# cloneofsimo/paint-with-words-sd

Hardware: NVIDIA H100
Metric: unet_steps_per_sec_512sq_cfg (higher is better)
Workload: dtype f16

## Files before the change

paint_with_words_sd_b200/csrc/pww_abi.cu:

```cuda
#include <stdio.h>
#include <string.h>

#include "pww_common.cuh"
#include "xattn_tc.cuh"
#include "xattn_fused2.cuh"
#include "attn_tc.cuh"
#include "unet_ops.cuh"
#include "sampler_step.cuh"
#include "control_inject.cuh"
#include "control_combine.cuh"
#include <stdlib.h>
#include <algorithm>
#include <type_traits>

namespace {

thread_local char g_last_cuda_error[640] = "";

int cuda_fail(cudaError_t e);

bool aligned16(const void* p) { return (reinterpret_cast<uintptr_t>(p) & 15u) == 0; }

bool supported_head_dim(int D) { return D == 40 || D == 64 || D == 80 || D == 160; }

// ... 143 lines not shown
              int64_t q_batch_stride, int64_t q_row_stride, int64_t k_batch_stride, int64_t k_row_stride,
              int64_t o_batch_stride, int64_t o_row_stride, const float* wmap, int64_t wmap_batch_stride,
              const int32_t* wmap_index, const float* stats, const float* g_sigma, int64_t g_stride, float scale,
              void* stream) {
  int rc = check_common(q, k, B, H, N, T, D, q_batch_stride, q_row_stride, k_batch_stride, k_row_stride);
  if (rc) return rc;
  if (!v || !out || !aligned16(v) || !aligned16(out)) return PWW_ERR_BAD_ARG;
  if ((o_batch_stride | o_row_stride) & 7 || o_row_stride < (int64_t)H * D) return PWW_ERR_BAD_ARG;
  if (wmap && (!stats || !g_sigma)) return PWW_ERR_BAD_ARG;
  pww::XattnParams<E> p = xattn_params<E>(q, k, v, out, B, H, N, T, D, q_batch_stride, q_row_stride, k_batch_stride,
                                          k_row_stride, o_batch_stride, o_row_stride);
  p.wmap = wmap; p.wmap_bs = wmap_batch_stride; p.wmap_index = wmap ? wmap_index : nullptr;
  p.stats = stats; p.g_sigma = g_sigma; p.g_stride = g_stride; p.scale = scale;
  for (int b0 = 0; b0 < B; b0 += pww::tc::kMaxBatch) {
    pww::XattnParams<E> c = images(p, b0, std::min(B - b0, pww::tc::kMaxBatch));
    if (wmap && !wmap_index) c.wmap += (int64_t)b0 * wmap_batch_stride;
    const cudaError_t e =
        with_shape(D, T, [&](auto k) { return pww::tc::launch_fwd<k.D, k.KC>(c, (cudaStream_t)stream); });
    if (e != cudaSuccess) return cuda_fail(e);
  }
  return PWW_OK;
}

template <typename E>
int xattn_fused(const void* q, const void* k, const void* v, void* out, int B, int H, int N, int T, int D,
                int64_t q_batch_stride, int64_t q_row_stride, int64_t k_batch_stride, int64_t k_row_stride,
                int64_t o_batch_stride, int64_t o_row_stride, const void* mpack, int64_t mpack_batch_stride, int Bw,
                const int8_t* cidx, const int32_t* wmap_index, int stat, const int32_t* kinds, bool per_image,
                const float* g_sigma, float scale, float* stats, void* workspace, size_t workspace_bytes,
                void* stream) {
  int rc = check_common(q, k, B, H, N, T, D, q_batch_stride, q_row_stride, k_batch_stride, k_row_stride);
  if (rc) return rc;
  if (!v || !out || !aligned16(v) || !aligned16(out)) return PWW_ERR_BAD_ARG;
  if ((o_batch_stride | o_row_stride) & 7 || o_row_stride < (int64_t)H * D || o_batch_stride <= 0) return PWW_ERR_BAD_ARG;
  if (mpack) {
    if (!cidx || !g_sigma || !workspace || Bw <= 0 || !aligned16(mpack)) return PWW_ERR_BAD_ARG;
    if ((mpack_batch_stride & 7) || mpack_batch_stride < (int64_t)N * pww::fx::kMW) return PWW_ERR_BAD_ARG;
    if (per_image ? !kinds : (stat != PWW_STAT_MAX && stat != PWW_STAT_STD)) return PWW_ERR_BAD_ARG;
    if (workspace_bytes < pww_xattn_fused_workspace_bytes()) return PWW_ERR_WORKSPACE;
  }
  pww::XattnParams<E> p = xattn_params<E>(q, k, v, out, B, H, N, T, D, q_batch_stride, q_row_stride, k_batch_stride,
                                          k_row_stride, o_batch_stride, o_row_stride);
  p.g_sigma = g_sigma; p.g_stride = per_image ? 1 : 0; p.scale = scale; p.stat = stat;
  p.stat_kind = per_image ? kinds : nullptr; p.stats_out = stats;
  p.wmap_index = mpack ? wmap_index : nullptr;
  p.counters = (unsigned int*)workspace;
  p.partials = workspace ? (pww::StatPartial*)((char*)workspace + 512) : nullptr;
  int chunk = pww::fx::kMaxBatch;
  const int tiles = pww::ceil_div(N, pww::core::kBM);
  const int hg = pww::ceil_div(H, D == 40 ? pww::fx::Cfg2<40>::G : (D == 64 ? pww::fx::Cfg2<64>::G : 1));
  while (chunk > 1) {
    const int cb = B < chunk ? B : chunk;
    if (pww::fx::fused2_fits(cb, hg, tiles, pww::fx::fused_grid(cb * hg * tiles))) break;
    chunk >>= 1;
  }
  for (int b0 = 0; b0 < B; b0 += chunk) {
    pww::XattnParams<E> c = images(p, b0, std::min(B - b0, chunk));
    const void* mp = mpack;
    const int8_t* ci = cidx;
    if (mpack && !wmap_index) {
      mp = (const __half*)mpack + (int64_t)b0 * mpack_batch_stride;
      ci = cidx + (int64_t)b0 * pww::core::kTP * pww::core::chunks_of(T);
    }
    c.wmap = (const float*)mp;
    const cudaError_t e = with_shape(D, T, [&](auto k) {
      return pww::fx::launch_fused2<k.D, k.KC>(c, mp, mpack_batch_stride, ci, (cudaStream_t)stream);
    });
    if (e == cudaErrorInvalidConfiguration) return PWW_ERR_UNSUPPORTED;
    if (e != cudaSuccess) return cuda_fail(e);
  }
  return PWW_OK;
}

template <typename E>
int groupnorm_nhwc(const void* x, const void* add, int64_t add_batch_stride, const void* gamma, const void* beta, void* y,
                   int B, int HW, int C, int G, float eps, int silu, void* workspace, size_t workspace_bytes,
                   void* stream) {
  if (!x || !gamma || !beta || !y || !workspace || B <= 0 || HW <= 0 || C <= 0 || G <= 0) return PWW_ERR_BAD_ARG;
  if (!aligned16(x) || !aligned16(y) || !aligned16(gamma) || !aligned16(beta) || (add && !aligned16(add)))
    return PWW_ERR_BAD_ARG;
  if ((C & 7) || (C % G) || G > 64 || (C >> 3) > 1024) return PWW_ERR_UNSUPPORTED;
  if (add && ((add_batch_stride & 7) || add_batch_stride < C)) return PWW_ERR_BAD_ARG;
  if (workspace_bytes < pww_groupnorm_workspace_bytes(B, HW, G)) return PWW_ERR_WORKSPACE;
  pww::uops::GnParams<E> p;
  p.x = (const E*)x; p.add = (const E*)add; p.add_bs = add_batch_stride; p.gamma = (const E*)gamma; p.beta = (const E*)beta;
  p.y = (E*)y;
  char* w = (char*)workspace;
  p.counters = (unsigned int*)w;
  w += align_up((size_t)B * sizeof(unsigned int), 256);
  p.stats = (float*)w;
  w += align_up((size_t)B * G * 2 * sizeof(float), 256);
  p.partial = (float*)w;
  p.B = B; p.HW = HW; p.C = C; p.G = G; p.eps = eps; p.silu = silu;
  p.chunks = pww::uops::gn_chunks(HW);
  p.rows_per_chunk = (HW + p.chunks - 1) / p.chunks;
  cudaStream_t s = (cudaStream_t)stream;
  const int nvec = C >> 3;
  const int rpp = nvec >= 256 ? 1 : 256 / nvec;
  const size_t smem1 = (size_t)rpp * C * 2 * sizeof(float);
  if (smem1 > 48 * 1024) return PWW_ERR_UNSUPPORTED;
  pww::uops::gn_stats_kernel<E><<<dim3(p.chunks, B), nvec * rpp, smem1, s>>>(p);
  int rows_per_block = (int)(((long long)HW * B + 2 * pww::num_sms() - 1) / (2 * pww::num_sms()));
  if (rows_per_block < rpp) rows_per_block = rpp;
  if (rows_per_block > 32) rows_per_block = 32;
  pww::uops::gn_apply_kernel<E><<<dim3((HW + rows_per_block - 1) / rows_per_block, B), nvec * rpp, 0, s>>>(p, rows_per_block);
  cudaError_t e = cudaGetLastError();
  return e == cudaSuccess ? PWW_OK : cuda_fail(e);
}

template <typename E>
int geglu(const void* in, void* out, int64_t M, int I, void* stream) {
  if (!in || !out || M <= 0 || I <= 0 || !aligned16(in) || !aligned16(out)) return PWW_ERR_BAD_ARG;
  if (I & 7) return PWW_ERR_UNSUPPORTED;
  const long long total = (long long)M * (I >> 3);
  long long blocks = (total + 255) / 256;
  const long long cap = (long long)pww::num_sms() * 16;
  if (blocks > cap) blocks = cap;
  pww::uops::geglu_kernel<E><<<(int)blocks, 256, 0, (cudaStream_t)stream>>>((const E*)in, (E*)out, M, I);
  cudaError_t e = cudaGetLastError();
  return e == cudaSuccess ? PWW_OK : cuda_fail(e);
}

template <typename E>
int add_layernorm(const void* x, const void* res, const void* gamma, const void* beta, void* sum_out, void* y, int64_t M,
                  int C, float eps, void* stream) {
  if (!x || !gamma || !beta || !y || M <= 0 || C <= 0) return PWW_ERR_BAD_ARG;
  if (!aligned16(x) || !aligned16(y) || !aligned16(gamma) || !aligned16(beta) || (res && !aligned16(res)) ||
      (sum_out && !aligned16(sum_out)))
    return PWW_ERR_BAD_ARG;
  if ((C & 7) || C > 2048) return PWW_ERR_UNSUPPORTED;
  const int warps = 8;
  const unsigned grid = (unsigned)((M + warps - 1) / warps);
  with_int<1, 8>(((C >> 3) + 31) / 32, [&](auto vpl) {
    pww::uops::add_layernorm_kernel<E, vpl><<<grid, warps * 32, 0, (cudaStream_t)stream>>>(
        (const E*)x, (const E*)res, (const E*)gamma, (const E*)beta, (E*)sum_out, (E*)y, M, C, eps);
  });
  cudaError_t e = cudaGetLastError();
  return e == cudaSuccess ? PWW_OK : cuda_fail(e);
}

template <typename E>
int resnet_residual(const void* a, const void* h, const float* bias, void* out, int64_t rows, int C, void* stream) {
  if (!a || !h || !bias || !out || rows <= 0 || C <= 0 || (C & 7)) return PWW_ERR_BAD_ARG;
  if (!aligned16(a) || !aligned16(h) || !aligned16(bias) || !aligned16(out)) return PWW_ERR_BAD_ARG;
  const long long total = (long long)rows * (C >> 3);
  long long blocks = (total + 255) / 256;
  const long long cap = (long long)pww::num_sms() * 16;
  if (blocks > cap) blocks = cap;
  pww::uops::resnet_residual_kernel<E><<<(int)blocks, 256, 0, (cudaStream_t)stream>>>(
      (const E*)a, (const E*)h, bias, (E*)out, total, C >> 3);
  cudaError_t e = cudaGetLastError();
  return e == cudaSuccess ? PWW_OK : cuda_fail(e);
}

template <typename E>
int attn_fwd(const void* q,const void* k, const void* v, void* out, int B, int H, int N, int D, int64_t qkv_batch_stride,
             int64_t qkv_row_stride, int64_t o_batch_stride, int64_t o_row_stride, float scale, void* stream) {
  if (!q || !k || !v || !out || B <= 0 || H <= 0 || N <= 0 || D <= 0) return PWW_ERR_BAD_ARG;
  if (!aligned16(q) || !aligned16(k) || !aligned16(v) || !aligned16(out)) return PWW_ERR_BAD_ARG;
  if ((qkv_batch_stride | qkv_row_stride | o_batch_stride | o_row_stride) & 7) return PWW_ERR_BAD_ARG;
  if (qkv_row_stride < (int64_t)H * D || o_row_stride < (int64_t)H * D) return PWW_ERR_BAD_ARG;
  if (!supported_head_dim(D)) return PWW_ERR_UNSUPPORTED;
  const cudaError_t e = with_shape(D, 1, [&](auto sh) {
    return pww::fa::launch<sh.D, E>(q, k, v, out, B, H, N, qkv_batch_stride, qkv_row_stride, o_batch_stride,
                                    o_row_stride, scale, (cudaStream_t)stream);
  });
  return e == cudaSuccess ? PWW_OK : cuda_fail(e);
}

template <typename E>
int control_inject(int n, void* const* dst, const void* const* res, const int64_t* elems_per_image, int rows,
                   const float* scales, void* stream) {
  if (n < 1 || n > pww::ctl::kMaxLevels || rows < 1 || !dst || !res || !elems_per_image) return PWW_ERR_BAD_ARG;
  pww::ctl::InjectArgs a;
  a.off[0] = 0;
  for (int k = 0; k < n; ++k) {
    const int64_t e = elems_per_image[k];
    if (e <= 0 || (e % pww::ctl::kVec) != 0) return PWW_ERR_BAD_ARG;
    if (!dst[k] || !res[k] || !aligned16(dst[k]) || !aligned16(res[k])) return PWW_ERR_BAD_ARG;
    a.dst[k] = dst[k];
    a.res[k] = res[k];
    a.vec_per_image[k] = e / pww::ctl::kVec;
    a.off[k + 1] = a.off[k] + (int64_t)rows * a.vec_per_image[k];
  }
  for (int k = n; k < pww::ctl::kMaxLevels; ++k) {
    a.dst[k] = nullptr;
    a.res[k] = nullptr;
    a.vec_per_image[k] = 0;
    a.off[k + 1] = a.off[n];
// ... 76 lines not shown
}
int pww_xattn_fwd_bf16(const void* q, const void* k, const void* v, void* out, int B, int H, int N, int T, int D,
    int64_t q_batch_stride, int64_t q_row_stride, int64_t k_batch_stride, int64_t k_row_stride, int64_t o_batch_stride,
    int64_t o_row_stride, const float* wmap, int64_t wmap_batch_stride, const int32_t* wmap_index, const float* stats,
    const float* g_sigma, float scale, void* stream) {
  return xattn_fwd<__nv_bfloat16>(
      q, k, v, out, B, H, N, T, D, q_batch_stride, q_row_stride, k_batch_stride, k_row_stride,
      o_batch_stride, o_row_stride, wmap, wmap_batch_stride, wmap_index, stats, g_sigma, 0, scale, stream);
}

int pww_xattn_fwd_multi_f16(const void* q, const void* k, const void* v, void* out, int B, int H, int N, int T, int D,
    int64_t q_batch_stride, int64_t q_row_stride, int64_t k_batch_stride, int64_t k_row_stride, int64_t o_batch_stride,
    int64_t o_row_stride, const float* wmap, int64_t wmap_batch_stride, const int32_t* wmap_index, const float* stats,
    const float* g_sigma, float scale, void* stream) {
  return xattn_fwd<__half>(q, k, v, out, B, H, N, T, D, q_batch_stride, q_row_stride, k_batch_stride, k_row_stride,
      o_batch_stride, o_row_stride, wmap, wmap_batch_stride, wmap_index, stats, g_sigma, 1, scale, stream);
}
int pww_xattn_fwd_multi_bf16(const void* q, const void* k, const void* v, void* out, int B, int H, int N, int T, int D,
    int64_t q_batch_stride, int64_t q_row_stride, int64_t k_batch_stride, int64_t k_row_stride, int64_t o_batch_stride,
    int64_t o_row_stride, const float* wmap, int64_t wmap_batch_stride, const int32_t* wmap_index, const float* stats,
    const float* g_sigma, float scale, void* stream) {
  return xattn_fwd<__nv_bfloat16>(
      q, k, v, out, B, H, N, T, D, q_batch_stride, q_row_stride, k_batch_stride, k_row_stride,
      o_batch_stride, o_row_stride, wmap, wmap_batch_stride, wmap_index, stats, g_sigma, 1, scale, stream);
}

size_t pww_xattn_fused_workspace_bytes(void) { return pww::fx::fused_workspace_bytes(); }

int pww_xattn_fused_f16(const void* q, const void* k, const void* v, void* out, int B, int H, int N, int T, int D,
    int64_t q_batch_stride, int64_t q_row_stride, int64_t k_batch_stride, int64_t k_row_stride, int64_t o_batch_stride,
    int64_t o_row_stride, const void* mpack, int64_t mpack_batch_stride, int Bw, const int8_t* cidx,
    const int32_t* wmap_index, int stat, const float* g_sigma, float scale, float* stats, void* workspace,
    size_t workspace_bytes, void* stream) {
  return xattn_fused<__half>(q, k, v, out, B, H, N, T, D, q_batch_stride, q_row_stride, k_batch_stride, k_row_stride,
      o_batch_stride, o_row_stride, mpack, mpack_batch_stride, Bw, cidx, wmap_index, stat, nullptr, false,
      g_sigma, scale, stats, workspace, workspace_bytes, stream);
}
int pww_xattn_fused_bf16(const void* q, const void* k, const void* v, void* out, int B, int H, int N, int T, int D,
    int64_t q_batch_stride, int64_t q_row_stride, int64_t k_batch_stride, int64_t k_row_stride, int64_t o_batch_stride,
    int64_t o_row_stride, const void* mpack, int64_t mpack_batch_stride, int Bw, const int8_t* cidx,
    const int32_t* wmap_index, int stat, const float* g_sigma, float scale, float* stats, void* workspace,
    size_t workspace_bytes, void* stream) {
  return xattn_fused<__nv_bfloat16>(
      q, k, v, out, B, H, N, T, D, q_batch_stride, q_row_stride, k_batch_stride, k_row_stride,
      o_batch_stride, o_row_stride, mpack, mpack_batch_stride, Bw, cidx, wmap_index, stat, nullptr, false,
      g_sigma, scale, stats, workspace, workspace_bytes, stream);
}

int pww_xattn_fused_multi_f16(const void* q, const void* k, const void* v, void* out, int B, int H, int N, int T, int D,
    int64_t q_batch_stride, int64_t q_row_stride, int64_t k_batch_stride, int64_t k_row_stride, int64_t o_batch_stride,
    int64_t o_row_stride, const void* mpack, int64_t mpack_batch_stride, int Bw, const int8_t* cidx,
    const int32_t* wmap_index, const int32_t* stat, const float* g_sigma, float scale, float* stats, void* workspace,
    size_t workspace_bytes, void* stream) {
  return xattn_fused<__half>(q, k, v, out, B, H, N, T, D, q_batch_stride, q_row_stride, k_batch_stride, k_row_stride,
      o_batch_stride, o_row_stride, mpack, mpack_batch_stride, Bw, cidx, wmap_index, PWW_STAT_MAX, stat, true,
      g_sigma, scale, stats, workspace, workspace_bytes, stream);
}
int pww_xattn_fused_multi_bf16(const void* q, const void* k, const void* v, void* out, int B, int H, int N, int T, int D,
    int64_t q_batch_stride, int64_t q_row_stride, int64_t k_batch_stride, int64_t k_row_stride, int64_t o_batch_stride,
    int64_t o_row_stride, const void* mpack, int64_t mpack_batch_stride, int Bw, const int8_t* cidx,
    const int32_t* wmap_index, const int32_t* stat, const float* g_sigma, float scale, float* stats, void* workspace,
    size_t workspace_bytes, void* stream) {
  return xattn_fused<__nv_bfloat16>(
      q, k, v, out, B, H, N, T, D, q_batch_stride, q_row_stride, k_batch_stride, k_row_stride,
      o_batch_stride, o_row_stride, mpack, mpack_batch_stride, Bw, cidx, wmap_index, PWW_STAT_MAX, stat, true,
      g_sigma, scale, stats, workspace, workspace_bytes, stream);
}

int pww_attn_fwd_f16(const void* q, const void* k, const void* v, void* out, int B, int H, int N, int D,
    int64_t qkv_batch_stride, int64_t qkv_row_stride, int64_t o_batch_stride, int64_t o_row_stride, float scale,
    void* stream) {
  return attn_fwd<__half>(
      q, k, v, out, B, H, N, D, qkv_batch_stride, qkv_row_stride, o_batch_stride, o_row_stride, scale, stream);
}
int pww_attn_fwd_bf16(const void* q, const void* k, const void* v, void* out, int B, int H, int N, int D,
    int64_t qkv_batch_stride, int64_t qkv_row_stride, int64_t o_batch_stride, int64_t o_row_stride, float scale,
    void* stream) {
  return attn_fwd<__nv_bfloat16>(
      q, k, v, out, B, H, N, D, qkv_batch_stride, qkv_row_stride, o_batch_stride, o_row_stride, scale, stream);
}

size_t pww_groupnorm_workspace_bytes(int B, int HW, int G) {
  if (B <= 0 || HW <= 0 || G <= 0) return 0;
  return align_up((size_t)B * sizeof(unsigned int), 256) + align_up((size_t)B * G * 2 * sizeof(float), 256) +
         (size_t)B * pww::uops::gn_chunks(HW) * G * 2 * sizeof(float);
}

int pww_groupnorm_nhwc_f16(const void* x, const void* add, int64_t add_batch_stride, const void* gamma,
    const void* beta, void* y, int B, int HW, int C, int G, float eps, int silu, void* workspace, size_t workspace_bytes,
    void* stream) {
  return groupnorm_nhwc<__half>(
      x, add, add_batch_stride, gamma, beta, y, B, HW, C, G, eps, silu, workspace, workspace_bytes,
      stream);
}
int pww_groupnorm_nhwc_bf16(const void* x, const void* add, int64_t add_batch_stride, const void* gamma,
    const void* beta, void* y, int B, int HW, int C, int G, float eps, int silu, void* workspace, size_t workspace_bytes,
    void* stream) {
  return groupnorm_nhwc<__nv_bfloat16>(
      x, add, add_batch_stride, gamma, beta, y, B, HW, C, G, eps, silu, workspace, workspace_bytes,
      stream);
}

int pww_geglu_f16(const void* in, void* out, int64_t M, int I, void* stream) {
  return geglu<__half>(in, out, M, I, stream);
}
int pww_geglu_bf16(const void* in, void* out, int64_t M, int I, void* stream) {
  return geglu<__nv_bfloat16>(in, out, M, I, stream);
}

int pww_add_layernorm_f16(const void* x, const void* res, const void* gamma, const void* beta, void* sum_out, void* y,
    int64_t M, int C, float eps, void* stream) {
  return add_layernorm<__half>(x, res, gamma, beta, sum_out, y, M, C, eps, stream);
}
int pww_add_layernorm_bf16(const void* x, const void* res, const void* gamma, const void* beta, void* sum_out, void* y,
    int64_t M, int C, float eps, void* stream) {
  return add_layernorm<__nv_bfloat16>(x, res, gamma, beta, sum_out, y, M, C, eps, stream);
}

int pww_resnet_residual_f16(const void* a, const void* h, const float* bias, void* out, int64_t rows, int C,
                            void* stream) {
  return resnet_residual<__half>(a, h, bias, out, rows, C, stream);
}
int pww_resnet_residual_bf16(const void* a, const void* h, const float* bias, void* out, int64_t rows, int C,
                             void* stream) {
  return resnet_residual<__nv_bfloat16>(a, h, bias, out, rows, C, stream);
}

int pww_sampler_input(const float* latents, const float* scale, const float* extra, void* out, int out_dtype, int m,
                      int channels, int height, int width, void* stream) {
  if (!latents || !scale || !out || m <= 0 || height <= 0 || width <= 0) return PWW_ERR_BAD_ARG;
  if (channels != 4 && channels != 9) return PWW_ERR_BAD_ARG;
  if ((channels == 9) != (extra != nullptr)) return PWW_ERR_BAD_ARG;
  if (out_dtype != PWW_DTYPE_F32 && out_dtype != PWW_DTYPE_F16 && out_dtype != PWW_DTYPE_BF16) return PWW_ERR_UNSUPPORTED;
  pww::smp::InputArgs a;
  a.lat = latents; a.scale = scale; a.extra = extra; a.out = out; a.m = m; a.C = channels; a.hw = height * width;
  const bool px4 = (a.hw % 4) == 0 && aligned16(latents) && (!extra || aligned16(extra)) && aligned16(out);
  cudaStream_t s = (cudaStream_t)stream;
  const cudaError_t e = out_dtype == PWW_DTYPE_F16    ? pww::smp::launch_input<__half>(a, px4, s)
                        : out_dtype == PWW_DTYPE_BF16 ? pww::smp::launch_input<__nv_bfloat16>(a, px4, s)
                                                      : pww::smp::launch_input<float>(a, px4, s);
  return e == cudaSuccess ? PWW_OK : cuda_fail(e);
}

int pww_sampler_update(const void* eps, int eps_dtype, int64_t eps_batch_stride, int64_t eps_channel_stride,
                       int64_t eps_row_stride, int64_t eps_col_stride, float* latents, float* history, int history_len,
                       const float* noise, const float* guidance, const float* beta, const float* form, int m,
                       int height, int width, void* stream) {
  if (!eps || !latents || !history || !guidance || !beta || !form) return PWW_ERR_BAD_ARG;
  if (m <= 0 || height <= 0 || width <= 0 || history_len < 1 || history_len > 4) return PWW_ERR_BAD_ARG;
  if (eps_dtype != PWW_DTYPE_F32 && eps_dtype != PWW_DTYPE_F16 && eps_dtype != PWW_DTYPE_BF16) return PWW_ERR_UNSUPPORTED;
  pww::smp::UpdateArgs a;
  a.eps = eps; a.e_sn = eps_batch_stride; a.e_sc = eps_channel_stride; a.e_sh = eps_row_stride; a.e_sw = eps_col_stride;
  a.lat = latents; a.hist = history; a.noise = noise; a.gscale = guidance; a.beta = beta; a.form = form;
  a.m = m; a.h = height; a.w = width; a.nh = history_len;
  const int64_t hw = (int64_t)height * width;
  const size_t es = eps_dtype == PWW_DTYPE_F32 ? 4 : 2;
  const bool px4 = (hw % 4) == 0 && aligned16(latents) && aligned16(history) && (!noise || aligned16(noise));
  const size_t need = px4 ? 16 : 4 * es;
  const bool cl = eps_channel_stride == 1 && eps_col_stride == 4 && eps_row_stride == 4 * (int64_t)width &&
                  (reinterpret_cast<uintptr_t>(eps) % need) == 0 && ((size_t)eps_batch_stride * es) % need == 0;
  cudaStream_t s = (cudaStream_t)stream;
  const cudaError_t e = eps_dtype == PWW_DTYPE_F16    ? pww::smp::launch_update<__half>(a, px4, cl, s)
                        : eps_dtype == PWW_DTYPE_BF16 ? pww::smp::launch_update<__nv_bfloat16>(a, px4, cl, s)
                                                      : pww::smp::launch_update<float>(a, px4, cl, s);
  return e == cudaSuccess ? PWW_OK : cuda_fail(e);
}

int pww_control_inject_f16(int n, void* const* dst, const void* const* res, const int64_t* elems_per_image, int rows,
// ... 42 lines not shown
```

paint_with_words_sd_b200/csrc/unet_ops.cuh:

```cuda
#pragma once
#include "pww_common.cuh"

namespace pww {
namespace uops {

template <typename E>
struct GnParams {
  const E* x;
  const E* add;
  long long add_bs;
  const E* gamma;
  const E* beta;
  E* y;
  float* partial;
  float* stats;
  unsigned int* counters;
  int B, HW, C, G, chunks, rows_per_chunk, silu;
  float eps;
};

template <typename E>
__global__ void gn_stats_kernel(GnParams<E> p) {
  using X = Elem<E>;
  using E2 = typename X::E2;
  extern __shared__ float sm[];
  const int nvec = p.C >> 3;
  const int rpp = blockDim.x / nvec;
  const int v = threadIdx.x % nvec, rl = threadIdx.x / nvec;
  const int b = blockIdx.y, chunk = blockIdx.x;
  const int r0 = chunk * p.rows_per_chunk, r1 = min(p.HW, r0 + p.rows_per_chunk);
  float s[8], q[8], a[8];
#pragma unroll
  for (int i = 0; i < 8; ++i) { s[i] = 0.f; q[i] = 0.f; a[i] = 0.f; }
  if (p.add) {
    const uint4 av = *reinterpret_cast<const uint4*>(p.add + (size_t)b * p.add_bs + v * 8);
    const E2* ah = reinterpret_cast<const E2*>(&av);
#pragma unroll
    for (int i = 0; i < 4; ++i) { float2 f = X::to_float2(ah[i]); a[2 * i] = f.x; a[2 * i + 1] = f.y; }
  }
  const E* xb = p.x + (size_t)b * p.HW * p.C;
  for (int r = r0 + rl; r < r1; r += 4 * rpp) {
    uint4 xv[4];
#pragma unroll
    for (int u = 0; u < 4; ++u) {
      const int rr = r + u * rpp;
      xv[u] = rr < r1 ? __ldg(reinterpret_cast<const uint4*>(xb + (size_t)rr * p.C) + v) : make_uint4(0, 0, 0, 0);
    }
#pragma unroll
    for (int u = 0; u < 4; ++u) {
      if (r + u * rpp < r1) {
        const E2* xh = reinterpret_cast<const E2*>(&xv[u]);
#pragma unroll
        for (int i = 0; i < 4; ++i) {
          float2 f = X::to_float2(xh[i]);
          const float x0 = f.x + a[2 * i], x1 = f.y + a[2 * i + 1];
          s[2 * i] += x0; q[2 * i] = fmaf(x0, x0, q[2 * i]);
          s[2 * i + 1] += x1; q[2 * i + 1] = fmaf(x1, x1, q[2 * i + 1]);
        }
      }
    }
  }
  float* ss = sm;
  float* sq = sm + rpp * p.C;
#pragma unroll
  for (int i = 0; i < 8; ++i) { ss[rl * p.C + v * 8 + i] = s[i]; sq[rl * p.C + v * 8 + i] = q[i]; }
  __syncthreads();
  const int cg = p.C / p.G;
  for (int g = threadIdx.x; g < p.G; g += blockDim.x) {
    float ts = 0.f, tq = 0.f;
    for (int r = 0; r < rpp; ++r)
      for (int c = g * cg; c < (g + 1) * cg; ++c) { ts += ss[r * p.C + c]; tq += sq[r * p.C + c]; }
    float* out = p.partial + (((size_t)b * p.chunks + chunk) * p.G + g) * 2;
    out[0] = ts; out[1] = tq;
  }
  __shared__ int is_last;
  __threadfence();
  __syncthreads();
  if (threadIdx.x == 0) is_last = (atomicAdd(&p.counters[b], 1u) == (unsigned)p.chunks - 1u) ? 1 : 0;
  __syncthreads();
  if (!is_last) return;
  __threadfence();
  const int warp = threadIdx.x >> 5, lane = threadIdx.x & 31, nwarps = blockDim.x >> 5;
  for (int g = warp; warp < nwarps && g < p.G; g += nwarps) {
    const float* pp = p.partial + ((size_t)b * p.chunks * p.G + g) * 2;
    float ts = 0.f, tq = 0.f;
    for (int c = lane; c < p.chunks; c += 32) { ts += __ldcg(pp + (size_t)c * p.G * 2); tq += __ldcg(pp + (size_t)c * p.G * 2 + 1); }
#pragma unroll
    for (int o = 16; o > 0; o >>= 1) {
      ts += __shfl_xor_sync(0xffffffffu, ts, o);
      tq += __shfl_xor_sync(0xffffffffu, tq, o);
    }
    if (lane == 0) {
      const float n = (float)p.HW * (float)cg;
      const float mean = ts / n;
      float var = tq / n - mean * mean;
      var = var < 0.f ? 0.f : var;
      p.stats[((size_t)b * p.G + g) * 2] = mean;
      p.stats[((size_t)b * p.G + g) * 2 + 1] = rsqrtf(var + p.eps);
    }
  }
  if (threadIdx.x == 0) p.counters[b] = 0u;
}

template <typename E>
__global__ void gn_apply_kernel(GnParams<E> p, int rows_per_block) {
  using X = Elem<E>;
  using E2 = typename X::E2;
  const int nvec = p.C >> 3;
  const int rpp = blockDim.x / nvec;
  const int v = threadIdx.x % nvec, rl = threadIdx.x / nvec;
  const int b = blockIdx.y;
  const int cg = p.C / p.G;
  float sc[8], sh[8];
  {
    const uint4 gv = __ldg(reinterpret_cast<const uint4*>(p.gamma) + v);
    const uint4 bv = __ldg(reinterpret_cast<const uint4*>(p.beta) + v);
    uint4 av = make_uint4(0, 0, 0, 0);
    if (p.add) av = __ldg(reinterpret_cast<const uint4*>(p.add + (size_t)b * p.add_bs) + v);
    const E* gh = reinterpret_cast<const E*>(&gv);
    const E* bh = reinterpret_cast<const E*>(&bv);
    const E* ah = reinterpret_cast<const E*>(&av);
#pragma unroll
    for (int i = 0; i < 8; ++i) {
      const int g = (v * 8 + i) / cg;
      const float mean = __ldg(p.stats + ((size_t)b * p.G + g) * 2), rstd = __ldg(p.stats + ((size_t)b * p.G + g) * 2 + 1);
      sc[i] = rstd * X::to_float(gh[i]);
      sh[i] = X::to_float(bh[i]) + (X::to_float(ah[i]) - mean) * sc[i];
    }
  }
  const int r0 = blockIdx.x * rows_per_block, r1 = min(p.HW, r0 + rows_per_block);
  const E* xb = p.x + (size_t)b * p.HW * p.C;
  E* yb = p.y + (size_t)b * p.HW * p.C;
  for (int r = r0 + rl; r < r1; r += rpp) {
    const uint4 xv = __ldg(reinterpret_cast<const uint4*>(xb + (size_t)r * p.C) + v);
    const E2* xh = reinterpret_cast<const E2*>(&xv);
    __align__(16) E2 o[4];
#pragma unroll
    for (int k = 0; k < 4; ++k) {
      const float2 f = X::to_float2(xh[k]);
      float y0 = fmaf(f.x, sc[2 * k], sh[2 * k]);
      float y1 = fmaf(f.y, sc[2 * k + 1], sh[2 * k + 1]);
      if (p.silu) {
        y0 = __fdividef(y0, 1.f + __expf(-y0));
        y1 = __fdividef(y1, 1.f + __expf(-y1));
      }
      o[k] = X::from_float2(y0, y1);
    }
    reinterpret_cast<uint4*>(yb + (size_t)r * p.C)[v] = *reinterpret_cast<const uint4*>(o);
  }
}

template <typename E>
__global__ void geglu_kernel(const E* __restrict__ in, E* __restrict__ out, long long M, int I) {
  using X = Elem<E>;
  using E2 = typename X::E2;
  const int nvec = I >> 3;
  const long long total = M * nvec;
  for (long long i = (long long)blockIdx.x * blockDim.x + threadIdx.x; i < total; i += (long long)gridDim.x * blockDim.x) {
    const long long m = i / nvec;
    const int v = (int)(i % nvec);
    const uint4 av = __ldg(reinterpret_cast<const uint4*>(in + m * 2 * I) + v);
    const uint4 gv = __ldg(reinterpret_cast<const uint4*>(in + m * 2 * I + I) + v);
    const E2* ah = reinterpret_cast<const E2*>(&av);
    const E2* gh = reinterpret_cast<const E2*>(&gv);
    __align__(16) E2 o[4];
#pragma unroll
    for (int k = 0; k < 4; ++k) {
      const float2 a = X::to_float2(ah[k]), g = X::to_float2(gh[k]);
      const float g0 = 0.5f * g.x * (1.f + erff(g.x * 0.70710678118654752f));
      const float g1 = 0.5f * g.y * (1.f + erff(g.y * 0.70710678118654752f));
      o[k] = X::from_float2(a.x * g0, a.y * g1);
    }
    reinterpret_cast<uint4*>(out + m * I)[v] = *reinterpret_cast<const uint4*>(o);
  }
}

template <typename E, int VPL>
__global__ void add_layernorm_kernel(const E* __restrict__ x, const E* __restrict__ res,
                                     const E* __restrict__ gamma, const E* __restrict__ beta,
                                     E* __restrict__ sum_out, E* __restrict__ y, long long M, int C, float eps) {
  using X = Elem<E>;
  using E2 = typename X::E2;
  const int lane = threadIdx.x & 31;
  const long long row = (long long)blockIdx.x * (blockDim.x >> 5) + (threadIdx.x >> 5);
  if (row >= M) return;
  const int nvec = C >> 3;
  float v[VPL][8];
  float sum = 0.f;
#pragma unroll
  for (int i = 0; i < VPL; ++i) {
    const int vi = lane + i * 32;
    if (vi < nvec) {
      const uint4 xv = __ldg(reinterpret_cast<const uint4*>(x + row * C) + vi);
      const E2* xh = reinterpret_cast<const E2*>(&xv);
      uint4 rv = make_uint4(0, 0, 0, 0);
      if (res) rv = __ldg(reinterpret_cast<const uint4*>(res + row * C) + vi);
      const E2* rh = reinterpret_cast<const E2*>(&rv);
      __align__(16) E2 so[4];
#pragma unroll
      for (int k = 0; k < 4; ++k) {
        const float2 a = X::to_float2(xh[k]), b = X::to_float2(rh[k]);
        so[k] = X::from_float2(a.x + b.x, a.y + b.y);
        const float2 f = X::to_float2(so[k]);
        v[i][2 * k] = f.x; v[i][2 * k + 1] = f.y;
        sum += f.x + f.y;
      }
      if (sum_out) reinterpret_cast<uint4*>(sum_out + row * C)[vi] = *reinterpret_cast<const uint4*>(so);
    } else {
#pragma unroll
      for (int k = 0; k < 8; ++k) v[i][k] = 0.f;
    }
  }
#pragma unroll
  for (int o = 16; o > 0; o >>= 1) sum += __shfl_xor_sync(0xffffffffu, sum, o);
  const float mean = sum / (float)C;
  float sq = 0.f;
#pragma unroll
  for (int i = 0; i < VPL; ++i) {
    if (lane + i * 32 < nvec) {
#pragma unroll
      for (int k = 0; k < 8; ++k) { const float d = v[i][k] - mean; sq = fmaf(d, d, sq); }
    }
  }
#pragma unroll
  for (int o = 16; o > 0; o >>= 1) sq += __shfl_xor_sync(0xffffffffu, sq, o);
  const float rstd = rsqrtf(sq / (float)C + eps);
#pragma unroll
  for (int i = 0; i < VPL; ++i) {
    const int vi = lane + i * 32;
    if (vi < nvec) {
      const uint4 gv = __ldg(reinterpret_cast<const uint4*>(gamma) + vi);
      const uint4 bv = __ldg(reinterpret_cast<const uint4*>(beta) + vi);
      const E2* gh = reinterpret_cast<const E2*>(&gv);
      const E2* bh = reinterpret_cast<const E2*>(&bv);
      __align__(16) E2 o[4];
#pragma unroll
      for (int k = 0; k < 4; ++k) {
        const float2 g = X::to_float2(gh[k]), b = X::to_float2(bh[k]);
        o[k] = X::from_float2((v[i][2 * k] - mean) * rstd * g.x + b.x, (v[i][2 * k + 1] - mean) * rstd * g.y + b.y);
      }
      reinterpret_cast<uint4*>(y + row * C)[vi] = *reinterpret_cast<const uint4*>(o);
    }
  }
}

template <typename E>
__global__ void resnet_residual_kernel(const E* a, const E* h, const float* __restrict__ bias, E* out,
                                       long long total_vec, int nvec) {
  using X = Elem<E>;
  using E2 = typename X::E2;
  for (long long i = (long long)blockIdx.x * blockDim.x + threadIdx.x; i < total_vec;
       i += (long long)gridDim.x * blockDim.x) {
    const int v = (int)(i % nvec);
    const uint4 av = reinterpret_cast<const uint4*>(a)[i];
    const uint4 hv = reinterpret_cast<const uint4*>(h)[i];
    const float4 b0 = __ldg(reinterpret_cast<const float4*>(bias) + 2 * v);
    const float4 b1 = __ldg(reinterpret_cast<const float4*>(bias) + 2 * v + 1);
    const float bb[8] = {b0.x, b0.y, b0.z, b0.w, b1.x, b1.y, b1.z, b1.w};
    const E2* ah = reinterpret_cast<const E2*>(&av);
    const E2* hh = reinterpret_cast<const E2*>(&hv);
    __align__(16) E2 o[4];
#pragma unroll
    for (int k = 0; k < 4; ++k) {
      const float2 fa = X::to_float2(ah[k]), fh = X::to_float2(hh[k]);
      o[k] = X::from_float2(fa.x + fh.x + bb[2 * k], fa.y + fh.y + bb[2 * k + 1]);
    }
    reinterpret_cast<uint4*>(out)[i] = *reinterpret_cast<const uint4*>(o);
  }
}

inline int gn_chunks(int HW) {
  int rows = HW >= 4096 ? 64 : (HW >= 1024 ? 32 : 16);
  int c = (HW + rows - 1) / rows;
  return c < 1 ? 1 : (c > 512 ? 512 : c);
}

}
}
```

paint_with_words_sd_b200/fused_ops.py:

```python
from __future__ import annotations

import ctypes
from typing import Dict, Optional

import torch

from . import _native

_WS: Dict[torch.device, torch.Tensor] = {}


def _workspace(device, nbytes: int) -> torch.Tensor:
    w = _WS.get(device)
    if w is None or w.numel() < nbytes:
        if w is not None:
            _WS_KEEP.append(w)
        w = torch.zeros(max(nbytes, 4 << 20), dtype=torch.uint8, device=device)
        _WS[device] = w
    return w


_WS_KEEP: list = []


ENABLED = True


def is_fast(x: torch.Tensor) -> bool:
    return ENABLED and x.is_cuda and x.dtype in (torch.float16, torch.bfloat16)


def group_norm_nhwc(x: torch.Tensor, gn: torch.nn.GroupNorm, add: Optional[torch.Tensor] = None,
                    silu: bool = True) -> torch.Tensor:
    if not x.is_contiguous(memory_format=torch.channels_last):
        x = x.contiguous(memory_format=torch.channels_last)
    B, C, H, W = x.shape
    L = _native.lib()
    y = torch.empty_like(x, memory_format=torch.channels_last)
    nbytes = L.pww_groupnorm_workspace_bytes(B, H * W, gn.num_groups)
    ws = _workspace(x.device, nbytes)
    add_bs = 0
    if add is not None:
        if add.dtype != x.dtype or add.stride(-1) != 1 or (add.stride(0) % 8) or (add.data_ptr() % 16):
            add = add.to(x.dtype).contiguous()
        add_bs = add.stride(0)
    fn = _native.entry("pww_groupnorm_nhwc", x.dtype)
    with torch.cuda.device(x.device):
        rc = fn(x.data_ptr(), None if add is None else add.data_ptr(), add_bs, gn.weight.data_ptr(),
                gn.bias.data_ptr(), y.data_ptr(), B, H * W, C, gn.num_groups, float(gn.eps),
                1 if silu else 0, ws.data_ptr(), ws.numel(), torch.cuda.current_stream(x.device).cuda_stream)
    _native.check(rc, fn.__name__)
    _native.launch_count += 2
    return y


def geglu(h: torch.Tensor) -> torch.Tensor:
    if not h.is_contiguous():
        h = h.contiguous()
    I = h.shape[-1] // 2
    M = h.numel() // h.shape[-1]
    out = torch.empty(h.shape[:-1] + (I,), dtype=h.dtype, device=h.device)
    fn = _native.entry("pww_geglu", h.dtype)
    with torch.cuda.device(h.device):
        rc = fn(h.data_ptr(), out.data_ptr(), M, I, torch.cuda.current_stream(h.device).cuda_stream)
    _native.check(rc, fn.__name__)
    _native.launch_count += 1
    return out


def add_layer_norm(x: torch.Tensor, res: Optional[torch.Tensor], ln: torch.nn.LayerNorm, want_sum: bool = True):
    if not x.is_contiguous():
        x = x.contiguous()
    if res is not None and not res.is_contiguous():
        res = res.contiguous()
    C = x.shape[-1]
    M = x.numel() // C
    y = torch.empty_like(x)
    s = torch.empty_like(x) if (res is not None and want_sum) else None
    fn = _native.entry("pww_add_layernorm", x.dtype)
    with torch.cuda.device(x.device):
        rc = fn(x.data_ptr(), None if res is None else res.data_ptr(), ln.weight.data_ptr(), ln.bias.data_ptr(),
                None if s is None else s.data_ptr(), y.data_ptr(), M, C, float(ln.eps),
                torch.cuda.current_stream(x.device).cuda_stream)
    _native.check(rc, fn.__name__)
    _native.launch_count += 1
    return (x if res is None else s), y


def resnet_residual(a: torch.Tensor, h: torch.Tensor, bias: torch.Tensor, out: Optional[torch.Tensor] = None):
    cl = torch.channels_last
    a, h = a.contiguous(memory_format=cl), h.contiguous(memory_format=cl)
    out = h if out is None else out
    C = h.shape[1]
    if (tuple(a.shape) != tuple(h.shape) or tuple(out.shape) != tuple(h.shape) or a.dtype != h.dtype
            or out.dtype != h.dtype or not all(t.is_contiguous(memory_format=cl) for t in (a, h, out))):
        raise ValueError(f"resnet_residual needs a, h and out of one shape and type, channels-last (got "
                         f"{tuple(a.shape)} {a.dtype}, {tuple(h.shape)} {h.dtype}, {tuple(out.shape)} {out.dtype})")
    if bias.dtype != torch.float32 or tuple(bias.shape) != (C,) or not bias.is_contiguous() or bias.device != h.device:
        raise ValueError(f"resnet_residual bias must be a contiguous fp32 [{C}] tensor on {h.device}")
    fn = _native.entry("pww_resnet_residual", h.dtype)
# ... 70 lines not shown
```

Measured before the change: 152.0.

## Restructure GroupNorm into channel-sliced stats and apply kernels with PDL

Rewrites the NHWC GroupNorm so both kernels split channels into slices over a 3D grid. Finalisation moves out of the last-block atomic counter in the stats kernel and into each apply block, which reduces the per-chunk partials itself. Stats accumulate around a per-group shift for numerical stability, loads are software-pipelined, and the apply kernel launches with programmatic dependent launch so its prologue overlaps the stats kernel. The workspace shrinks and is no longer zeroed. The cost is that every apply block re-reduces the partials, and the indexing is more complex.

```diff
diff --git a/paint_with_words_sd_b200/csrc/pww_abi.cu b/paint_with_words_sd_b200/csrc/pww_abi.cu
--- a/paint_with_words_sd_b200/csrc/pww_abi.cu
+++ b/paint_with_words_sd_b200/csrc/pww_abi.cu
@@ -249,29 +249,33 @@
   if ((C & 7) || (C % G) || G > 64 || (C >> 3) > 1024) return PWW_ERR_UNSUPPORTED;
   if (add && ((add_batch_stride & 7) || add_batch_stride < C)) return PWW_ERR_BAD_ARG;
   if (workspace_bytes < pww_groupnorm_workspace_bytes(B, HW, G)) return PWW_ERR_WORKSPACE;
+  const pww::uops::GnSplit sp = pww::uops::gn_split(HW, C, G);
   pww::uops::GnParams<E> p;
   p.x = (const E*)x; p.add = (const E*)add; p.add_bs = add_batch_stride; p.gamma = (const E*)gamma; p.beta = (const E*)beta;
   p.y = (E*)y;
-  char* w = (char*)workspace;
-  p.counters = (unsigned int*)w;
-  w += align_up((size_t)B * sizeof(unsigned int), 256);
-  p.stats = (float*)w;
-  w += align_up((size_t)B * G * 2 * sizeof(float), 256);
-  p.partial = (float*)w;
-  p.B = B; p.HW = HW; p.C = C; p.G = G; p.eps = eps; p.silu = silu;
-  p.chunks = pww::uops::gn_chunks(HW);
-  p.rows_per_chunk = (HW + p.chunks - 1) / p.chunks;
+  p.partial = (float2*)workspace;
+  p.HW = HW; p.C = C; p.G = G; p.eps = eps; p.silu = silu;
+  p.sv = sp.sv; p.chunks = sp.chunks; p.rows_per_chunk = sp.rows_per_chunk;
   cudaStream_t s = (cudaStream_t)stream;
-  const int nvec = C >> 3;
-  const int rpp = nvec >= 256 ? 1 : 256 / nvec;
-  const size_t smem1 = (size_t)rpp * C * 2 * sizeof(float);
-  if (smem1 > 48 * 1024) return PWW_ERR_UNSUPPORTED;
-  pww::uops::gn_stats_kernel<E><<<dim3(p.chunks, B), nvec * rpp, smem1, s>>>(p);
-  int rows_per_block = (int)(((long long)HW * B + 2 * pww::num_sms() - 1) / (2 * pww::num_sms()));
-  if (rows_per_block < rpp) rows_per_block = rpp;
-  if (rows_per_block > 32) rows_per_block = 32;
-  pww::uops::gn_apply_kernel<E><<<dim3((HW + rows_per_block - 1) / rows_per_block, B), nvec * rpp, 0, s>>>(p, rows_per_block);
-  cudaError_t e = cudaGetLastError();
+  const size_t smem1 = (64 + (size_t)2 * sp.rpp * sp.sv * 8) * sizeof(float);
+  if (smem1 > 48 * 1024) {
+    const cudaError_t e = pww::allow_dynamic_smem<pww::uops::gn_stats_kernel<E>>(64 * 1024 + 256);
+    if (e != cudaSuccess) return cuda_fail(e);
+  }
+  pww::uops::gn_stats_kernel<E><<<dim3(sp.chunks, sp.slices, B), sp.threads, smem1, s>>>(p);
+  int rows = 4;
+  while (rows > 1 && (long long)B * sp.slices * pww::ceil_div(HW, sp.rpp * rows) < 2 * pww::num_sms()) rows >>= 1;
+  cudaLaunchAttribute pdl;
+  pdl.id = cudaLaunchAttributeProgrammaticStreamSerialization;
+  pdl.val.programmaticStreamSerializationAllowed = 1;
+  cudaLaunchConfig_t cfg = {};
+  cfg.gridDim = dim3(pww::ceil_div(HW, sp.rpp * rows), sp.slices, B);
+  cfg.blockDim = dim3(sp.threads);
+  cfg.stream = s;
+  cfg.attrs = &pdl;
+  cfg.numAttrs = 1;
+  cudaError_t e = cudaLaunchKernelEx(&cfg, pww::uops::gn_apply_kernel<E>, p, sp.rpp * rows);
+  if (e == cudaSuccess) e = cudaGetLastError();
   return e == cudaSuccess ? PWW_OK : cuda_fail(e);
 }
 
@@ -514,8 +518,8 @@
 
 size_t pww_groupnorm_workspace_bytes(int B, int HW, int G) {
   if (B <= 0 || HW <= 0 || G <= 0) return 0;
-  return align_up((size_t)B * sizeof(unsigned int), 256) + align_up((size_t)B * G * 2 * sizeof(float), 256) +
-         (size_t)B * pww::uops::gn_chunks(HW) * G * 2 * sizeof(float);
+  const size_t chunks = (size_t)std::min(HW, pww::uops::kGnMaxChunks);
+  return align_up((size_t)B * G * chunks * sizeof(float2), 256);
 }
 
 int pww_groupnorm_nhwc_f16(const void* x, const void* add, int64_t add_batch_stride, const void* gamma,
diff --git a/paint_with_words_sd_b200/csrc/unet_ops.cuh b/paint_with_words_sd_b200/csrc/unet_ops.cuh
--- a/paint_with_words_sd_b200/csrc/unet_ops.cuh
+++ b/paint_with_words_sd_b200/csrc/unet_ops.cuh
@@ -12,128 +12,162 @@
   const E* gamma;
   const E* beta;
   E* y;
-  float* partial;
-  float* stats;
-  unsigned int* counters;
-  int B, HW, C, G, chunks, rows_per_chunk, silu;
+  float2* partial;
+  int HW, C, G, sv, chunks, rows_per_chunk, silu;
   float eps;
 };
 
 template <typename E>
-__global__ void gn_stats_kernel(GnParams<E> p) {
-  using X = Elem<E>;
-  using E2 = typename X::E2;
+__device__ __forceinline__ float gn_shift(const GnParams<E>& p, int b, int c) {
+  float s = Elem<E>::to_float(p.x[(size_t)b * p.HW * p.C + c]);
+  if (p.add) s += Elem<E>::to_float(p.add[(size_t)b * p.add_bs + c]);
+  return s;
+}
+
+__device__ __forceinline__ void gn_load4(uint4 (&xv)[4], const uint4* col, int stride_vec, int r, int rpp, int r1) {
+#pragma unroll
+  for (int u = 0; u < 4; ++u) {
+    const int rr = r + u * rpp;
+    xv[u] = rr < r1 ? __ldg(col + (size_t)rr * stride_vec) : make_uint4(0, 0, 0, 0);
+  }
+}
+
+template <typename E>
+__global__ void __launch_bounds__(1024) gn_stats_kernel(GnParams<E> p) {
+  using X = Elem<E>;
+  using E2 = typename X::E2;
+  asm volatile("griddepcontrol.launch_dependents;" ::: "memory");
   extern __shared__ float sm[];
-  const int nvec = p.C >> 3;
-  const int rpp = blockDim.x / nvec;
-  const int v = threadIdx.x % nvec, rl = threadIdx.x / nvec;
-  const int b = blockIdx.y, chunk = blockIdx.x;
-  const int r0 = chunk * p.rows_per_chunk, r1 = min(p.HW, r0 + p.rows_per_chunk);
-  float s[8], q[8], a[8];
-#pragma unroll
-  for (int i = 0; i < 8; ++i) { s[i] = 0.f; q[i] = 0.f; a[i] = 0.f; }
-  if (p.add) {
-    const uint4 av = *reinterpret_cast<const uint4*>(p.add + (size_t)b * p.add_bs + v * 8);
+  const int cg = p.C / p.G, sv = p.sv, rpp = blockDim.x / sv, b = blockIdx.z;
+  const int v0 = blockIdx.y * sv, nv = min(sv, (p.C >> 3) - v0);
+  const int c0 = v0 * 8, ng = nv * 8 / cg;
+  const int v = threadIdx.x % sv, rl = threadIdx.x / sv;
+  const bool lane_on = rl < rpp && v < nv;
+  const int r0 = blockIdx.x * p.rows_per_chunk;
+  const int r1 = lane_on ? min(p.HW, r0 + p.rows_per_chunk) : r0;
+  const uint4* col = reinterpret_cast<const uint4*>(p.x + (size_t)b * p.HW * p.C + c0) + v;
+  const int stride_vec = p.C >> 3;
+  uint4 xv[4];
+  gn_load4(xv, col, stride_vec, r0 + rl, rpp, r1);
+  float* s_shift = sm;
+  float* ss = sm + 64;
+  float* sq = ss + rpp * sv * 8;
+  if (threadIdx.x < ng) s_shift[threadIdx.x] = gn_shift(p, b, c0 + threadIdx.x * cg);
+  float o[8], s[8], q[8];
+#pragma unroll
+  for (int i = 0; i < 8; ++i) { o[i] = 0.f; s[i] = 0.f; q[i] = 0.f; }
+  if (p.add && lane_on) {
+    const uint4 av = __ldg(reinterpret_cast<const uint4*>(p.add + (size_t)b * p.add_bs + c0) + v);
     const E2* ah = reinterpret_cast<const E2*>(&av);
 #pragma unroll
-    for (int i = 0; i < 4; ++i) { float2 f = X::to_float2(ah[i]); a[2 * i] = f.x; a[2 * i + 1] = f.y; }
-  }
-  const E* xb = p.x + (size_t)b * p.HW * p.C;
+    for (int i = 0; i < 4; ++i) { const float2 f = X::to_float2(ah[i]); o[2 * i] = f.x; o[2 * i + 1] = f.y; }
+  }
+  __syncthreads();
+#pragma unroll
+  for (int i = 0; i < 8; ++i) o[i] -= s_shift[(v * 8 + i) / cg];
   for (int r = r0 + rl; r < r1; r += 4 * rpp) {
-    uint4 xv[4];
-#pragma unroll
-    for (int u = 0; u < 4; ++u) {
-      const int rr = r + u * rpp;
-      xv[u] = rr < r1 ? __ldg(reinterpret_cast<const uint4*>(xb + (size_t)rr * p.C) + v) : make_uint4(0, 0, 0, 0);
-    }
 #pragma unroll
     for (int u = 0; u < 4; ++u) {
       if (r + u * rpp < r1) {
         const E2* xh = reinterpret_cast<const E2*>(&xv[u]);
 #pragma unroll
         for (int i = 0; i < 4; ++i) {
-          float2 f = X::to_float2(xh[i]);
-          const float x0 = f.x + a[2 * i], x1 = f.y + a[2 * i + 1];
-          s[2 * i] += x0; q[2 * i] = fmaf(x0, x0, q[2 * i]);
-          s[2 * i + 1] += x1; q[2 * i + 1] = fmaf(x1, x1, q[2 * i + 1]);
+          const float2 f = X::to_float2(xh[i]);
+          const float d0 = f.x + o[2 * i], d1 = f.y + o[2 * i + 1];
+          s[2 * i] += d0; q[2 * i] = fmaf(d0, d0, q[2 * i]);
+          s[2 * i + 1] += d1; q[2 * i + 1] = fmaf(d1, d1, q[2 * i + 1]);
         }
       }
     }
-  }
-  float* ss = sm;
-  float* sq = sm + rpp * p.C;
-#pragma unroll
-  for (int i = 0; i < 8; ++i) { ss[rl * p.C + v * 8 + i] = s[i]; sq[rl * p.C + v * 8 + i] = q[i]; }
+    if (r + 4 * rpp < r1) gn_load4(xv, col, stride_vec, r + 4 * rpp, rpp, r1);
+  }
+  const int w8 = sv * 8;
+  if (lane_on) {
+#pragma unroll
+    for (int i = 0; i < 8; ++i) { ss[rl * w8 + v * 8 + i] = s[i]; sq[rl * w8 + v * 8 + i] = q[i]; }
+  }
   __syncthreads();
-  const int cg = p.C / p.G;
-  for (int g = threadIdx.x; g < p.G; g += blockDim.x) {
+  const int warp = threadIdx.x >> 5, lane = threadIdx.x & 31, nwarps = blockDim.x >> 5, n = rpp * cg;
+  for (int lg = warp; lg < ng; lg += nwarps) {
     float ts = 0.f, tq = 0.f;
-    for (int r = 0; r < rpp; ++r)
-      for (int c = g * cg; c < (g + 1) * cg; ++c) { ts += ss[r * p.C + c]; tq += sq[r * p.C + c]; }
-    float* out = p.partial + (((size_t)b * p.chunks + chunk) * p.G + g) * 2;
-    out[0] = ts; out[1] = tq;
-  }
-  __shared__ int is_last;
-  __threadfence();
+    for (int j = lane; j < n; j += 32) {
+      const int r = j / cg, c = lg * cg + (j - r * cg);
+      ts += ss[r * w8 + c]; tq += sq[r * w8 + c];
+    }
+#pragma unroll
+    for (int m = 16; m > 0; m >>= 1) {
+      ts += __shfl_xor_sync(0xffffffffu, ts, m);
+      tq += __shfl_xor_sync(0xffffffffu, tq, m);
+    }
+    if (lane == 0) p.partial[((size_t)b * p.G + c0 / cg + lg) * p.chunks + blockIdx.x] = make_float2(ts, tq);
+  }
+}
+
+template <typename E>
+__global__ void __launch_bounds__(1024) gn_apply_kernel(GnParams<E> p, int rows_per_block) {
+  using X = Elem<E>;
+  using E2 = typename X::E2;
+  __shared__ float2 s_stat[64];
+  const int cg = p.C / p.G, sv = p.sv, rpp = blockDim.x / sv, b = blockIdx.z;
+  const int v0 = blockIdx.y * sv, nv = min(sv, (p.C >> 3) - v0);
+  const int c0 = v0 * 8, ng = nv * 8 / cg;
+  const int v = threadIdx.x % sv, rl = threadIdx.x / sv;
+  const bool lane_on = rl < rpp && v < nv;
+  const int r0 = blockIdx.x * rows_per_block;
+  const int r1 = lane_on ? min(p.HW, r0 + rows_per_block) : r0;
+  const int stride_vec = p.C >> 3;
+  const uint4* __restrict__ xcol = reinterpret_cast<const uint4*>(p.x + (size_t)b * p.HW * p.C + c0) + v;
+  uint4* __restrict__ ycol = reinterpret_cast<uint4*>(p.y + (size_t)b * p.HW * p.C + c0) + v;
+  uint4 xv[4];
+  gn_load4(xv, xcol, stride_vec, r0 + rl, rpp, r1);
+  float sc[8], sh[8];
+  uint4 gv = make_uint4(0, 0, 0, 0), bv = gv, av = gv;
+  if (lane_on) {
+    gv = __ldg(reinterpret_cast<const uint4*>(p.gamma + c0) + v);
+    bv = __ldg(reinterpret_cast<const uint4*>(p.beta + c0) + v);
+    if (p.add) av = __ldg(reinterpret_cast<const uint4*>(p.add + (size_t)b * p.add_bs + c0) + v);
+  }
+  {
+    int L = 32;
+    while (ng * L > (int)blockDim.x) L >>= 1;
+    const int lg = threadIdx.x / L, j = threadIdx.x % L, g = c0 / cg + lg;
+    float ts = 0.f, tq = 0.f, shift = 0.f;
+    if (lg < ng && j == 0) shift = gn_shift(p, b, g * cg);
+    asm volatile("griddepcontrol.wait;" ::: "memory");
+    if (lg < ng) {
+      const float2* pp = p.partial + ((size_t)b * p.G + g) * p.chunks;
+#pragma unroll 4
+      for (int c = j; c < p.chunks; c += L) { const float2 t = pp[c]; ts += t.x; tq += t.y; }
+    }
+    for (int m = L >> 1; m > 0; m >>= 1) {
+      ts += __shfl_xor_sync(0xffffffffu, ts, m);
+      tq += __shfl_xor_sync(0xffffffffu, tq, m);
+    }
+    if (lg < ng && j == 0) {
+      const float n = (float)p.HW * (float)cg;
+      const float dm = ts / n;
+      float var = tq / n - dm * dm;
+      var = var < 0.f ? 0.f : var;
+      s_stat[lg] = make_float2(shift + dm, rsqrtf(var + p.eps));
+    }
+  }
   __syncthreads();
-  if (threadIdx.x == 0) is_last = (atomicAdd(&p.counters[b], 1u) == (unsigned)p.chunks - 1u) ? 1 : 0;
-  __syncthreads();
-  if (!is_last) return;
-  __threadfence();
-  const int warp = threadIdx.x >> 5, lane = threadIdx.x & 31, nwarps = blockDim.x >> 5;
-  for (int g = warp; warp < nwarps && g < p.G; g += nwarps) {
-    const float* pp = p.partial + ((size_t)b * p.chunks * p.G + g) * 2;
-    float ts = 0.f, tq = 0.f;
-    for (int c = lane; c < p.chunks; c += 32) { ts += __ldcg(pp + (size_t)c * p.G * 2); tq += __ldcg(pp + (size_t)c * p.G * 2 + 1); }
-#pragma unroll
-    for (int o = 16; o > 0; o >>= 1) {
-      ts += __shfl_xor_sync(0xffffffffu, ts, o);
-      tq += __shfl_xor_sync(0xffffffffu, tq, o);
-    }
-    if (lane == 0) {
-      const float n = (float)p.HW * (float)cg;
-      const float mean = ts / n;
-      float var = tq / n - mean * mean;
-      var = var < 0.f ? 0.f : var;
-      p.stats[((size_t)b * p.G + g) * 2] = mean;
-      p.stats[((size_t)b * p.G + g) * 2 + 1] = rsqrtf(var + p.eps);
-    }
-  }
-  if (threadIdx.x == 0) p.counters[b] = 0u;
-}
-
-template <typename E>
-__global__ void gn_apply_kernel(GnParams<E> p, int rows_per_block) {
-  using X = Elem<E>;
-  using E2 = typename X::E2;
-  const int nvec = p.C >> 3;
-  const int rpp = blockDim.x / nvec;
-  const int v = threadIdx.x % nvec, rl = threadIdx.x / nvec;
-  const int b = blockIdx.y;
-  const int cg = p.C / p.G;
-  float sc[8], sh[8];
   {
-    const uint4 gv = __ldg(reinterpret_cast<const uint4*>(p.gamma) + v);
-    const uint4 bv = __ldg(reinterpret_cast<const uint4*>(p.beta) + v);
-    uint4 av = make_uint4(0, 0, 0, 0);
-    if (p.add) av = __ldg(reinterpret_cast<const uint4*>(p.add + (size_t)b * p.add_bs) + v);
     const E* gh = reinterpret_cast<const E*>(&gv);
     const E* bh = reinterpret_cast<const E*>(&bv);
     const E* ah = reinterpret_cast<const E*>(&av);
 #pragma unroll
     for (int i = 0; i < 8; ++i) {
-      const int g = (v * 8 + i) / cg;
-      const float mean = __ldg(p.stats + ((size_t)b * p.G + g) * 2), rstd = __ldg(p.stats + ((size_t)b * p.G + g) * 2 + 1);
-      sc[i] = rstd * X::to_float(gh[i]);
-      sh[i] = X::to_float(bh[i]) + (X::to_float(ah[i]) - mean) * sc[i];
-    }
-  }
-  const int r0 = blockIdx.x * rows_per_block, r1 = min(p.HW, r0 + rows_per_block);
-  const E* xb = p.x + (size_t)b * p.HW * p.C;
-  E* yb = p.y + (size_t)b * p.HW * p.C;
-  for (int r = r0 + rl; r < r1; r += rpp) {
-    const uint4 xv = __ldg(reinterpret_cast<const uint4*>(xb + (size_t)r * p.C) + v);
-    const E2* xh = reinterpret_cast<const E2*>(&xv);
+      const float2 st = s_stat[(v * 8 + i) / cg];
+      sc[i] = st.y * X::to_float(gh[i]);
+      sh[i] = X::to_float(bh[i]) + (X::to_float(ah[i]) - st.x) * sc[i];
+    }
+  }
+  const int r = r0 + rl;
+#pragma unroll
+  for (int u = 0; u < 4; ++u) {
+    if (r + u * rpp >= r1) break;
+    const E2* xh = reinterpret_cast<const E2*>(&xv[u]);
     __align__(16) E2 o[4];
 #pragma unroll
     for (int k = 0; k < 4; ++k) {
@@ -146,7 +180,7 @@
       }
       o[k] = X::from_float2(y0, y1);
     }
-    reinterpret_cast<uint4*>(yb + (size_t)r * p.C)[v] = *reinterpret_cast<const uint4*>(o);
+    ycol[(size_t)(r + u * rpp) * stride_vec] = *reinterpret_cast<const uint4*>(o);
   }
 }
 
@@ -269,11 +303,33 @@
   }
 }
 
-inline int gn_chunks(int HW) {
-  int rows = HW >= 4096 ? 64 : (HW >= 1024 ? 32 : 16);
-  int c = (HW + rows - 1) / rows;
-  return c < 1 ? 1 : (c > 512 ? 512 : c);
-}
-
-}
-}
+constexpr int kGnMaxChunks = 64;
+constexpr int kGnStatBlocksPerImage = 128;
+struct GnSplit {
+  int sv;
+  int slices;
+  int threads, rpp;
+  int chunks, rows_per_chunk;
+};
+inline GnSplit gn_split(int HW, int C, int G) {
+  GnSplit s;
+  const int cg = C / G, nvec = C >> 3;
+  int gcd = cg, t = 8;
+  while (t) { const int r = gcd % t; gcd = t; t = r; }
+  const int uv = cg / gcd;
+  const int nunits = nvec / uv, want = (nvec + 31) / 32;
+  const int per_slice = (nunits + want - 1) / want;
+  s.sv = per_slice * uv;
+  s.slices = (nunits + per_slice - 1) / per_slice;
+  s.threads = s.sv > 256 ? (s.sv + 31) / 32 * 32 : 256;
+  s.rpp = s.threads / s.sv;
+  int chunks = (kGnStatBlocksPerImage + s.slices - 1) / s.slices;
+  const int most = (HW + s.rpp - 1) / s.rpp;
+  chunks = chunks < most ? chunks : most;
+  chunks = chunks < kGnMaxChunks ? chunks : kGnMaxChunks;
+  s.rows_per_chunk = (HW + chunks - 1) / chunks;
+  s.chunks = (HW + s.rows_per_chunk - 1) / s.rows_per_chunk;
+  return s;
+}
+}
+}
diff --git a/paint_with_words_sd_b200/fused_ops.py b/paint_with_words_sd_b200/fused_ops.py
--- a/paint_with_words_sd_b200/fused_ops.py
+++ b/paint_with_words_sd_b200/fused_ops.py
@@ -15,7 +15,7 @@
     if w is None or w.numel() < nbytes:
         if w is not None:
             _WS_KEEP.append(w)
-        w = torch.zeros(max(nbytes, 4 << 20), dtype=torch.uint8, device=device)
+        w = torch.empty(max(nbytes, 4 << 20), dtype=torch.uint8, device=device)
         _WS[device] = w
     return w
 
```

Result: faster. 160.9 (median of 6 runs) (+5.9%).
